# KangWelly/Assignment-for-AAE6102_GNSS-SDR

Hardware: NVIDIA B200
Metric: search cells/s (PRN x Doppler x code-phase), 32-PRN acquisition (higher is better)
Workload: dtype f32

## Files before the change

### assignment-for-aae6102_gnss-sdr_b200/csrc/gnss_kernels.cuh

```cuda
#pragma once
#include <cooperative_groups.h>
#include <climits>
#include "gnss_internal.h"

namespace gnss {
namespace cg = cooperative_groups;

struct NaturalLoader {
    static constexpr bool kStreams = false;
    const cf* __restrict__ in;
    template <int Q>
    __device__ __forceinline__ void load(int a, int b, cf (&z)[Q]) const {
        static_for<0, Q>([&](auto c_) {
            constexpr int C = decltype(c_)::value;
            z[C] = in[Geo<Q>::good(a, b, C)];
        });
    }
};
struct NaturalStorer {
    cf* __restrict__ out;
    template <int Q, int R>
    __device__ __forceinline__ void store2(int col, int, const cf (&w0)[16], const cf (&w1)[16]) {
        static_for<0, 16>([&](auto i_) {
            constexpr int I = decltype(i_)::value;
            constexpr int AP = (I / 4) + 4 * (I % 4);
            out[Geo<Q>::lag_of(AP, col)] = w0[I];
            if (col + 1 < Geo<Q>::ROW) out[Geo<Q>::lag_of(AP, col + 1)] = w1[I];
        });
    }
};

template <int R>
__device__ __forceinline__ void cl_arrive() {
    if constexpr (R > 1) asm volatile("barrier.cluster.arrive.release.aligned;" ::: "memory");
}
template <int R>
__device__ __forceinline__ void cl_wait() {
    if constexpr (R > 1) asm volatile("barrier.cluster.wait.acquire.aligned;" ::: "memory");
    else __syncthreads();
}
template <int R>
__device__ __forceinline__ void cl_sync() {
    cl_arrive<R>();
    cl_wait<R>();
}

template <int Q, int R, int T>
__device__ __forceinline__ void pass2_all(cf* D, const Tw4* tw, int tid) {
    pass2_cta<Q, R, T>(tid, D, tw);
}

template <int Q, int R, int T>
__device__ __forceinline__ void pass3_all(cf* D, const Tw4* tw, int tid) {
    using S = Split<Q, R>;
    (void)tw;
    for (int t = tid; t < S::P3_TASKS; t += T) pass3_task<Q, R>(t, D);
}

struct RedScratch {
    float wv[32];
    int wm[32];
    double ws[32];
    float peak; int lag; double sum_all; double sum_win;
    float g_peak; int g_lag;
};

template <int Q, int R>
struct Smem {
    using S = Split<Q, R>;
    static constexpr size_t d_bytes = (size_t)S::D_ELEMS * sizeof(cf);
    static constexpr size_t acc_floats = S::ACC_ELEMS > SplitX<Q, R>::ACC_ELEMS ? S::ACC_ELEMS : SplitX<Q, R>::ACC_ELEMS;
    static constexpr size_t acc_bytes = acc_floats * sizeof(float);
    static constexpr size_t tw_bytes = 100 * sizeof(Tw4);
    static constexpr size_t red_bytes = ((sizeof(RedScratch) + 15) / 16) * 16;
    static constexpr size_t transform = d_bytes + tw_bytes;
    static constexpr size_t search = d_bytes + acc_bytes + tw_bytes + red_bytes;
};

__device__ __forceinline__ void fill_tw125(Tw4* tw, int tid, int T) {
    for (int j = tid; j < 100; j += T) {
        double s, c;
        sincospi(-2.0 * (double)((j >> 2) * ((j & 3) + 1)) / 125.0, &s, &c);
        Tw4 w;
        w.c = (float)c; w.pad = 0.f; w.ns = -(float)s; w.s = (float)s;
        tw[j] = w;
    }
}

template <int T>
__device__ __forceinline__ void block_reduce(float& v, int& m, double& s, RedScratch* rs) {
    constexpr unsigned full = 0xffffffffu;
    constexpr int NW = T / 32;
#pragma unroll
    for (int off = 16; off; off >>= 1) {
        const float ov = __shfl_down_sync(full, v, off);
        const int om = __shfl_down_sync(full, m, off);
        const double os = __shfl_down_sync(full, s, off);
        if (peak_better(ov, om, v, m)) { v = ov; m = om; }
        s += os;
    }
    const int warp = threadIdx.x >> 5, lane = threadIdx.x & 31;
    if (lane == 0) { rs->wv[warp] = v; rs->wm[warp] = m; rs->ws[warp] = s; }
    __syncthreads();
    if (warp == 0) {
        v = lane < NW ? rs->wv[lane] : -1.f;
        m = lane < NW ? rs->wm[lane] : INT_MAX;
        s = lane < NW ? rs->ws[lane] : 0.0;
#pragma unroll
        for (int off = 16; off; off >>= 1) {
            const float ov = __shfl_down_sync(full, v, off);
            const int om = __shfl_down_sync(full, m, off);
            const double os = __shfl_down_sync(full, s, off);
            if (peak_better(ov, om, v, m)) { v = ov; m = om; }
            s += os;
        }
    }
    __syncthreads();
}

template <int Q, int R, int T, class Loader, class Storer>
__device__ __forceinline__ void unit_device(const Loader& ld, Storer& st, cf* D, cf* const* Dall,
                                            const Tw4* tw, int rank, int tid) {
    using S = Split<Q, R>;
    for (int t = tid; t < S::P1_TASKS; t += T) pass1_task<Q, R>(t, rank, ld, D);
    __syncthreads();
    pass2_all<Q, R, T>(D, tw, tid);
    __syncthreads();
    pass3_all<Q, R, T>(D, tw, tid);
    cl_sync<R>();
    for (int t = tid; t < S::P4_TASKS; t += T) pass4_task<Q, R>(t, rank, Dall, st);
    cl_sync<R>();
}

template <int Q, int R, int T, class Loader, class Storer>
__device__ __forceinline__ void unit_device_pipelined(const Loader& ld, Storer& st, cf* D, cf* const* Dall,
                                                      const Tw4* tw, int rank, int tid) {
    using S = Split<Q, R>;
    {
        cf z[Q];
        const bool has = tid < S::P1_TASKS;
        if (has) pass1_compute<Q, R>(tid, rank, ld, z);
        cl_wait<R>();
        if (has) pass1_store<Q, R>(tid, z, D);
    }
    for (int t = tid + T; t < S::P1_TASKS; t += T) pass1_task<Q, R>(t, rank, ld, D);
    __syncthreads();
    pass2_all<Q, R, T>(D, tw, tid);
    __syncthreads();
    pass3_all<Q, R, T>(D, tw, tid);
    cl_sync<R>();
    for (int t = tid; t < S::P4_TASKS; t += T) pass4_task<Q, R>(t, rank, Dall, st);
    cl_arrive<R>();
}

#define GNSS_KERNEL_PROLOGUE                                                     \
    using S = Split<Q, R>;                                                       \
    using G = Geo<Q>;                                                            \
    (void)sizeof(G);                                                             \
    cg::cluster_group cluster = cg::this_cluster();                              \
    const int tid = threadIdx.x;                                                 \
    const int rank = (R > 1) ? (int)cluster.block_rank() : 0;                    \
    const int unit = blockIdx.x / R;                                             \
    extern __shared__ __align__(16) unsigned char smem_raw[];                    \
    cf* D = reinterpret_cast<cf*>(smem_raw);                                     \
    cf* Dall[R];                                                                 \
    _Pragma("unroll") for (int r = 0; r < R; ++r)                                \
        Dall[r] = (R > 1) ? cluster.map_shared_rank(D, r) : D;

template <int Q, int R, int T, int MINB>
__global__ void __launch_bounds__(T, MINB) code_kernel(CodeArgs a) {
    GNSS_KERNEL_PROLOGUE
    Tw4* tw = reinterpret_cast<Tw4*>(D + S::D_ELEMS);
    fill_tw125(tw, tid, T);
    __syncthreads();
    CodeLoader ld{a.scode + (size_t)unit * G::N};
    SpectrumStorer st{a.cc + (size_t)unit * G::N, 1.0f / (float)G::N, 1, 0};
    unit_device<Q, R, T>(ld, st, D, Dall, tw, rank, tid);
}

template <int Q, int R, int T, int MINB>
__global__ void __launch_bounds__(T, MINB) wipe_kernel(WipeArgs a) {
    GNSS_KERNEL_PROLOGUE
    Tw4* tw = reinterpret_cast<Tw4*>(D + S::D_ELEMS);
    fill_tw125(tw, tid, T);
    __syncthreads();
    const int base = unit / a.K, k = unit - base * a.K;
    WipeoffLoader ld;
    ld.raw = (const unsigned char*)a.raw + (size_t)k * a.block_bytes;
    ld.data_type = a.data_type;
    ld.precision = a.precision;
    ld.coh_ms = a.coh_ms;
    ld.f_hz = a.base_freq_hz[base];
    ld.fs_hz = a.fs_hz;
    ld.mean_i = a.means ? (float)a.means[0] : 0.f;
    ld.mean_q = a.means ? (float)a.means[1] : 0.f;
    SpectrumStorer st{a.x + (size_t)unit * G::NX, 1.0f, 0, 1};
    unit_device<Q, R, T>(ld, st, D, Dall, tw, rank, tid);
}

__device__ __forceinline__ void cp_async16(void* smem_dst, const void* gmem_src) {
    const unsigned d = (unsigned)__cvta_generic_to_shared(smem_dst);
    asm volatile("cp.async.cg.shared.global [%0], [%1], 16;" ::"r"(d), "l"(gmem_src) : "memory");
}
__device__ __forceinline__ void cp_async_commit() { asm volatile("cp.async.commit_group;" ::: "memory"); }
template <int N_>
__device__ __forceinline__ void cp_async_wait() { asm volatile("cp.async.wait_group %0;" ::"n"(N_) : "memory"); }

template <int Q>
GNSS_HD int comb_row_of(int a) { return (a * (Geo<Q>::M1 % 16)) % 16; }

template <int Q, int R, int T, int MINB>
__global__ void __launch_bounds__(T, MINB) wipe2_kernel(Wipe2Args a) {
    GNSS_KERNEL_PROLOGUE
    Tw4* tw = reinterpret_cast<Tw4*>(D + S::D_ELEMS);
    unsigned char* stage = reinterpret_cast<unsigned char*>(tw + 100);
    fill_tw125(tw, tid, T);
    const int base = unit / a.K, k = unit - base * a.K;
    const double w = a.base_w[base];
    const float mean_i = a.means ? (float)a.means[0] : 0.f, mean_q = a.means ? (float)a.means[1] : 0.f;
    const int pitch = a.pitch, bps = a.bps, M = a.coh_ms;
    auto stage_ms = [&](int j, int buf) {
        const int chunks = pitch >> 4;
        for (int i = tid; i < S::A * chunks; i += T) {
            const int al = i / chunks, ch = i - al * chunks;
            const int rho = comb_row_of<Q>(rank * S::A + al);
            const unsigned char* src = a.comb + ((size_t)((size_t)k * M + j) * 16 + rho) * pitch + (size_t)ch * 16;
            cp_async16(stage + ((size_t)buf * S::A + al) * pitch + (size_t)ch * 16, src);
        }
        cp_async_commit();
    };
    constexpr int ROUNDS = (S::P1_TASKS + T - 1) / T;
    const int n_steps = (M > 1) ? ROUNDS * M : 1;
    stage_ms(0, 0);
    int step = 0;
    for (int t0 = 0; t0 < S::P1_TASKS; t0 += T) {
        const int task = t0 + tid;
        const bool has = task < S::P1_TASKS;
        const int al = has ? task / 125 : 0, b = has ? task - al * 125 : 0;
        const int arow = rank * S::A + al;
        cf z[Q];
        static_for<0, Q>([&](auto c_) { z[decltype(c_)::value] = mk(0.f, 0.f); });
        for (int j = 0; j < M; ++j) {
            const int buf = (M > 1) ? (step & 1) : 0;
            if (M > 1 || t0 == 0) {
                if (step + 1 < n_steps) { stage_ms((j + 1) % M, buf ^ 1); cp_async_wait<1>(); }
                else cp_async_wait<0>();
                __syncthreads();
            }
            if (has) {
                const unsigned char* row = stage + ((size_t)buf * S::A + al) * pitch;
                static_for<0, Q>([&](auto c_) {
                    constexpr int C = decltype(c_)::value;
                    const int n = Geo<Q>::good(arow, b, C);
                    const int m = n >> 4;
                    float xi, xq;
                    if (bps == 2) {
                        const unsigned short v = *reinterpret_cast<const unsigned short*>(row + 2 * m);
                        xi = (float)(signed char)(v & 0xff);
                        xq = (float)(signed char)(v >> 8);
                    } else if (bps == 4) {
                        const unsigned v = *reinterpret_cast<const unsigned*>(row + 4 * m);
                        xi = (float)(short)(v & 0xffff) - mean_i;
                        xq = (float)(short)(v >> 16) - mean_q;
                    } else {
                        xi = (float)(signed char)row[m];
                        xq = 0.f;
                    }
                    const double cyc = w * (double)((long long)j * Geo<Q>::N + n + 1);
                    const float fr = (float)(cyc - floor(cyc));
                    float si, co;
                    sincospif(2.0f * fr, &si, &co);
                    z[C].x += xi * co - xq * si;
                    z[C].y += xi * si + xq * co;
                });
            }
            if (M > 1) __syncthreads();
            ++step;
        }
        if (has) {
            dft_odd<Q>(z);
            pass1_store<Q, R>(task, z, D);
        }
    }
    cp_async_wait<0>();
    __syncthreads();
    pass2_all<Q, R, T>(D, tw, tid);
    __syncthreads();
    pass3_all<Q, R, T>(D, tw, tid);
    cl_sync<R>();
    SpectrumStorer st{a.x + (size_t)unit * G::NX, 1.0f, 0, 1};
    for (int t = tid; t < S::P4_TASKS; t += T) pass4_task<Q, R>(t, rank, Dall, st);
    cl_sync<R>();
}

template <int Q, int R, int T, int MINB>
__global__ void __launch_bounds__(T, MINB) natural_kernel(NaturalArgs a) {
    GNSS_KERNEL_PROLOGUE
    Tw4* tw = reinterpret_cast<Tw4*>(D + S::D_ELEMS);
    fill_tw125(tw, tid, T);
    __syncthreads();
    NaturalLoader ld{a.in + (size_t)unit * G::N};
    NaturalStorer st{a.out + (size_t)unit * G::N};
    unit_device<Q, R, T>(ld, st, D, Dall, tw, rank, tid);
}

template <int Q, int R, int T, int MINB>
__global__ void __launch_bounds__(T, MINB) fine_kernel(FineArgs a) {
    GNSS_KERNEL_PROLOGUE
    Tw4* tw = reinterpret_cast<Tw4*>(D + S::D_ELEMS);
    fill_tw125(tw, tid, T);
    __syncthreads();
    const int n2 = unit % a.L, r = (unit / a.L) % a.K, sv = unit / (a.L * a.K);
    FineLoader ld;
    ld.raw = a.raw;
    ld.chip = a.chip;
    ld.ca = a.ca + (size_t)sv * 1023;
    ld.data_type = a.data_type;
    ld.precision = a.precision;
    ld.mean_i = a.means ? (float)a.means[0] : 0.f;
    ld.mean_q = a.means ? (float)a.means[1] : 0.f;
    ld.start = a.start[sv];
    ld.L = a.L;
    ld.n2 = n2;
    ld.r = r;
    ld.F = a.F;
    NaturalStorerHD st{a.u + (size_t)unit * G::N};
    unit_device<Q, R, T>(ld, st, D, Dall, tw, rank, tid);
}

template <int Q, int R, int T, int MINB>
__global__ void __launch_bounds__(T, MINB) search_kernel(SearchArgs a) {
    GNSS_KERNEL_PROLOGUE
    float* acc = reinterpret_cast<float*>(D + S::D_ELEMS);
    Tw4* tw = reinterpret_cast<Tw4*>(acc + Smem<Q, R>::acc_floats);
    RedScratch* rs = reinterpret_cast<RedScratch*>(tw + 100);
    const int row = a.rows ? a.rows[unit] : a.row_first + unit;
    const int p = row % a.P, b = row / a.P;

    fill_tw125(tw, tid, T);
    for (int e = tid; e < S::ACC_ELEMS; e += T) acc[e] = 0.f;
    __syncthreads();

    int sa, sb, sc;
    G::shift_coords(a.bin_shift[b], sa, sb, sc);
    const cf* ccp = a.cc + (size_t)p * G::N;
    const cf* xb = a.x + (size_t)a.bin_base[b] * a.K * G::NX;
    PowerAccumStorer st{acc};
    cl_arrive<R>();
    for (int k = 0; k < a.K; ++k) {
        SearchLoader ld{ccp, xb + (size_t)k * G::NX, sa, sb, sc};
        unit_device_pipelined<Q, R, T>(ld, st, D, Dall, tw, rank, tid);
    }
    cl_wait<R>();

    float bv = -1.f;
    int bm = INT_MAX;
    double ss = 0.0;
    for (int e = tid; e < S::ACC_ELEMS; e += T) {
        const int ap = e / S::CH, t = e - ap * S::CH;
        const int col = rank * S::CH + t;
        if (col < S::ROW) {
            const float v = acc[e];
            const int m = G::lag_of(ap, col);
            if (peak_better(v, m, bv, bm)) { bv = v; bm = m; }
            ss += (double)v * (double)v;
            if (a.surface) a.surface[((size_t)p * a.B + b) * G::N + m] = v;
        }
    }
    block_reduce<T>(bv, bm, ss, rs);
    if (tid == 0) { rs->peak = bv; rs->lag = bm; rs->sum_all = ss; }
    if constexpr (R > 1) cluster.sync(); else __syncthreads();
    if (tid == 0) {
        float gv = -1.f;
        int gm = INT_MAX;
        for (int r = 0; r < R; ++r) {
            const RedScratch* o = (R > 1) ? cluster.map_shared_rank(rs, r) : rs;
            const float ov = o->peak;
            const int om = o->lag;
            if (peak_better(ov, om, gv, gm)) { gv = ov; gm = om; }
        }
        rs->g_peak = gv;
        rs->g_lag = gm;
    }
    __syncthreads();
    const int gm = rs->g_lag;
    double wsum = 0.0;
    for (int i = tid; i < 2 * a.w - 1; i += T) {
        const int m = gm - (a.w - 1) + i;
        if (m >= 0 && m < G::N) {
            int ap, col;
            G::cell_of_lag(m, ap, col);
            if (col / S::CH == rank) {
                const float v = acc[ap * S::CH + (col - rank * S::CH)];
                wsum += (double)v * (double)v;
            }
        }
    }
    float dv = -1.f;
    int dm = INT_MAX;
    block_reduce<T>(dv, dm, wsum, rs);
    if (tid == 0) rs->sum_win = wsum;
    if constexpr (R > 1) cluster.sync(); else __syncthreads();
    if (rank == 0 && tid == 0) {
        double s_all = 0.0, s_win = 0.0;
        for (int r = 0; r < R; ++r) {
            const RedScratch* o = (R > 1) ? cluster.map_shared_rank(rs, r) : rs;
            s_all += o->sum_all;
            s_win += o->sum_win;
        }
        Candidate c;
        c.peak = rs->g_peak;
        c.lag = rs->g_lag;
        c.sum_all = s_all;
        c.sum_win = s_win;
        a.cand[(size_t)p * a.cand_stride + b] = c;
    }
    if constexpr (R > 1) cluster.sync();
}

template <int Q, int R, int T, int MINB>
__global__ void __launch_bounds__(T, MINB) search_kernel_l2x(SearchArgs a) {
    GNSS_KERNEL_PROLOGUE
    (void)Dall;
    float* acc = reinterpret_cast<float*>(D + S::D_ELEMS);
    Tw4* tw = reinterpret_cast<Tw4*>(acc + Smem<Q, R>::acc_floats);
    RedScratch* rs = reinterpret_cast<RedScratch*>(tw + 100);
    const int ncl = gridDim.x / R, slot = unit;
    cf* xch = a.scratch + (size_t)slot * 2 * 16 * S::RS;
    fill_tw125(tw, tid, T);
    PowerAccumStorer st{acc};

    for (int lrow = slot; lrow < a.n_rows; lrow += ncl) {
        const int row = a.rows ? a.rows[lrow] : a.row_first + lrow;
        const int p = row % a.P, b = row / a.P;
        for (int e = tid; e < S::ACC_ELEMS; e += T) acc[e] = 0.f;
        int sa, sb, sc;
        G::shift_coords(a.bin_shift[b], sa, sb, sc);
        const cf* ccp = a.cc + (size_t)p * G::N;
        const cf* xb = a.x + (size_t)a.bin_base[b] * a.K * G::NX;
        {
            SearchLoader ld{ccp, xb, sa, sb, sc};
            for (int t = tid; t < S::P1_TASKS; t += T) pass1_task<Q, R>(t, rank, ld, D);
        }
        __syncthreads();
        pass2_all<Q, R, T>(D, tw, tid);
        __syncthreads();
        pass3_all<Q, R, T>(D, tw, tid);
        for (int k = 0; k < a.K; ++k) {
            const bool more = k + 1 < a.K;
            cf* buf = xch + (size_t)(k & 1) * 16 * S::RS;
            __syncthreads();
            {
                const float4* src = reinterpret_cast<const float4*>(D);
                float4* dst = reinterpret_cast<float4*>(buf + (size_t)rank * S::A * S::RS);
                for (int i = tid; i < S::D_ELEMS / 2; i += T) dst[i] = src[i];
            }
            if (more) {
                SearchLoader ld{ccp, xb + (size_t)(k + 1) * G::NX, sa, sb, sc};
                cf z[Q];
                const bool has = tid < S::P1_TASKS;
                if (has) pass1_compute<Q, R>(tid, rank, ld, z);
                __syncthreads();
                if (has) pass1_store<Q, R>(tid, z, D);
                for (int t = tid + T; t < S::P1_TASKS; t += T) pass1_task<Q, R>(t, rank, ld, D);
            }
            cl_arrive<R>();
            if (more) {
                __syncthreads();
                pass2_all<Q, R, T>(D, tw, tid);
            }
            cl_wait<R>();
            for (int t = tid; t < S::P4_TASKS; t += T) pass4_task_flat<Q, R>(t, rank, buf, st);
            if (more) {
                __syncthreads();
                pass3_all<Q, R, T>(D, tw, tid);
            }
        }
        __syncthreads();

        float bv = -1.f;
        int bm = INT_MAX;
        double ss = 0.0;
        for (int e = tid; e < S::ACC_ELEMS; e += T) {
            const int ap = e / S::CH, t = e - ap * S::CH;
            const int col = rank * S::CH + t;
            if (col < S::ROW) {
                const float v = acc[e];
                const int m = G::lag_of(ap, col);
                if (peak_better(v, m, bv, bm)) { bv = v; bm = m; }
                ss += (double)v * (double)v;
                if (a.surface) a.surface[((size_t)p * a.B + b) * G::N + m] = v;
            }
        }
        block_reduce<T>(bv, bm, ss, rs);
        if (tid == 0) { rs->peak = bv; rs->lag = bm; rs->sum_all = ss; }
        if constexpr (R > 1) cluster.sync(); else __syncthreads();
        if (tid == 0) {
            float gv = -1.f;
            int gm = INT_MAX;
            for (int r = 0; r < R; ++r) {
                const RedScratch* o = (R > 1) ? cluster.map_shared_rank(rs, r) : rs;
                const float ov = o->peak;
                const int om = o->lag;
                if (peak_better(ov, om, gv, gm)) { gv = ov; gm = om; }
            }
            rs->g_peak = gv;
            rs->g_lag = gm;
        }
        __syncthreads();
        const int gm = rs->g_lag;
        double wsum = 0.0;
        for (int i = tid; i < 2 * a.w - 1; i += T) {
            const int m = gm - (a.w - 1) + i;
            if (m >= 0 && m < G::N) {
                int ap, col;
                G::cell_of_lag(m, ap, col);
                if (col / S::CH == rank) {
                    const float v = acc[ap * S::CH + (col - rank * S::CH)];
                    wsum += (double)v * (double)v;
                }
            }
        }
        float dv = -1.f;
        int dm = INT_MAX;
        block_reduce<T>(dv, dm, wsum, rs);
        if (tid == 0) rs->sum_win = wsum;
        if constexpr (R > 1) cluster.sync(); else __syncthreads();
        if (rank == 0 && tid == 0) {
            double s_all = 0.0, s_win = 0.0;
            for (int r = 0; r < R; ++r) {
                const RedScratch* o = (R > 1) ? cluster.map_shared_rank(rs, r) : rs;
                s_all += o->sum_all;
                s_win += o->sum_win;
            }
            Candidate c;
            c.peak = rs->g_peak;
            c.lag = rs->g_lag;
            c.sum_all = s_all;
            c.sum_win = s_win;
            a.cand[(size_t)p * a.cand_stride + b] = c;
        }
        if constexpr (R > 1) cluster.sync(); else __syncthreads();
    }
}

__device__ __forceinline__ void group_arrive(unsigned* ctr) {
#ifdef GNSS_EXPERIMENT_NOFENCE
    asm volatile("red.relaxed.gpu.global.add.u32 [%0], 1;" ::"l"(ctr) : "memory");
#else
    asm volatile("red.release.gpu.global.add.u32 [%0], 1;" ::"l"(ctr) : "memory");
#endif
}
__device__ __forceinline__ void group_arrive_n(unsigned* ctr, unsigned n) {
    asm volatile("red.release.gpu.global.add.u32 [%0], %1;" ::"l"(ctr), "r"(n) : "memory");
}
__device__ __forceinline__ void group_spin(const unsigned* ctr, unsigned target) {
    unsigned v;
    do {
        asm volatile("ld.acquire.gpu.global.u32 %0, [%1];" : "=r"(v) : "l"(ctr) : "memory");
    } while ((int)(v - target) < 0);
}

template <int Q, int R, int T>
__device__ __noinline__ void publish_plane(float* acc, float* dst, int tid) {
    using SX = SplitX<Q, R>;
    for (int j = tid; j < SX::P4_TASKS; j += T) {
#pragma unroll
        for (int ap = 0; ap < 16; ++ap) {
            float2* p = reinterpret_cast<float2*>(acc + ap * SX::CHX + 2 * j);
            __stcg(reinterpret_cast<float2*>(dst + ap * SX::CHX + 2 * j), *p);
            *p = make_float2(0.f, 0.f);
        }
    }
}
template <int Q, int R, int T>
__device__ __noinline__ void merge_planes(float* acc, const float* planes, int n_planes, int tid) {
    constexpr int ACC4 = SplitX<Q, R>::ACC_ELEMS / 4;
    const float4* src = reinterpret_cast<const float4*>(planes);
    float4* a4 = reinterpret_cast<float4*>(acc);
    int q = tid;
    for (; q + T < ACC4; q += 2 * T) {
        float4 v = a4[q], w = a4[q + T];
#pragma unroll 4
        for (int k = 0; k < n_planes; ++k) {
            const float4 o = __ldcg(src + (size_t)k * (R * ACC4) + q);
            const float4 u = __ldcg(src + (size_t)k * (R * ACC4) + q + T);
            v.x += o.x; v.y += o.y; v.z += o.z; v.w += o.w;
            w.x += u.x; w.y += u.y; w.z += u.z; w.w += u.w;
        }
        a4[q] = v;
        a4[q + T] = w;
    }
    for (; q < ACC4; q += T) {
        float4 v = a4[q];
#pragma unroll 8
        for (int k = 0; k < n_planes; ++k) {
            const float4 o = __ldcg(src + (size_t)k * (R * ACC4) + q);
            v.x += o.x; v.y += o.y; v.z += o.z; v.w += o.w;
        }
        a4[q] = v;
    }
}

#ifdef GNSS_EXPERIMENT_NOBAR
#define GNSS_KSYNC() __syncwarp()
#else
#define GNSS_KSYNC() __syncthreads()
#endif
#ifdef GNSS_TIMELINE
#define GNSS_TL(i) do { if (tl_iter == 6 && group == 0 && (tid & 31) == 0) a.timeline[(rank * (T / 32) + (tid >> 5)) * 32 + (i)] = clock64(); } while (0)
#else
#define GNSS_TL(i) do { } while (0)
#endif
template <int Q, int R, int T, int MINB>
__global__ void __launch_bounds__(T, MINB) search_kernel_coop(SearchArgs a) {
    using S = Split<Q, R>;
    using G = Geo<Q>;
    using GX = GeoX<Q>;
    using SX = SplitX<Q, R>;
    const int tid = threadIdx.x;
    const int tid2 = (tid + T - 32) % T;
    const int tid3 = (tid + T - (64 % T)) % T;
    const int rank = blockIdx.x % R, group = blockIdx.x / R, ngroups = gridDim.x / R;
    extern __shared__ __align__(16) unsigned char smem_raw[];
    cf* D = reinterpret_cast<cf*>(smem_raw);
    float* acc = reinterpret_cast<float*>(D + S::D_ELEMS);
    Tw4* tw = reinterpret_cast<Tw4*>(acc + Smem<Q, R>::acc_floats);
    RedScratch* rs = reinterpret_cast<RedScratch*>(tw + 100);
    constexpr size_t XBUF = (size_t)16 * GX::RSX;
    cf* xch = a.scratch + (size_t)group * 2 * XBUF;
    unsigned* ctr = a.group_ctr + group;
    Candidate* slots = a.row_slots + (size_t)group * R;
    unsigned target = 0;
    fill_tw125(tw, tid, T);
    constexpr bool kRoomy = (T * MINB <= 512);
    constexpr bool kRegAcc = (Q <= 13) && kRoomy && (SX::P4_TASKS <= T);
    float racc0[16], racc1[16];
#pragma unroll
    for (int q = 0; q < 16; ++q) { racc0[q] = 0.f; racc1[q] = 0.f; }
    RegAccumStorer rst{racc0, racc1};
    PowerAccumStorer st{acc};
    auto dump_acc = [&]() {
        if constexpr (kRegAcc) {
            if (tid < SX::P4_TASKS) {
#pragma unroll
                for (int ap = 0; ap < 16; ++ap) {
                    *reinterpret_cast<float2*>(acc + ap * SX::CHX + 2 * tid) = make_float2(racc0[ap], racc1[ap]);
                    racc0[ap] = 0.f; racc1[ap] = 0.f;
                }
            }
        }
    };
    const int n_rows = a.n_rows;
    auto loader_of = [&](int lrow) {
        const int row = a.rows ? a.rows[lrow] : a.row_first + lrow;
        const int p = row % a.P, b = row / a.P;
        int sa, sb, sc;
        G::shift_coords(a.bin_shift[b], sa, sb, sc);
        return SearchLoader{a.cc + (size_t)p * G::N, a.x + (size_t)a.bin_base[b] * a.K * G::NX, sa, sb, sc};
    };
    const int full = n_rows / ngroups, tail_base = full * ngroups, n_tail = n_rows - tail_base;
    auto tb = [&](int g) -> int {
        return a.row_granular ? (g < n_tail ? g : n_tail) * a.K : (int)((unsigned)g * (unsigned)(n_tail * a.K) / (unsigned)ngroups);
    };
    struct Part { int row, kb, ke; };
    auto part = [&](int i) -> Part {
        if (i < full) return Part{i * ngroups + group, 0, a.K};
        const int t0 = tb(group), t1 = tb(group + 1), r0 = t0 / a.K, e0 = min(t1, (r0 + 1) * a.K);
        if (i == full) return Part{tail_base + r0, t0 - r0 * a.K, e0 - r0 * a.K};
        return Part{tail_base + r0 + 1, 0, t1 - e0};
    };
    auto count_parts = [&]() -> int {
        const int t0 = tb(group), t1 = tb(group + 1);
        return full + (t0 < t1 ? 1 + (min(t1, (t0 / a.K + 1) * a.K) < t1) : 0);
    };
    if (count_parts() == 0) return;
    int i = 0, par = 0;
    const Part first = part(0);
    int left = first.ke - first.kb;
    bool later = first.kb > 0;
    for (int e = tid; e < SX::ACC_ELEMS; e += T) acc[e] = 0.f;
    SearchLoader ld = loader_of(first.row);
    ld.x += (size_t)first.kb * G::NX;
    for (int t = tid; t < S::P1_TASKS; t += T) pass1_task<Q, R>(t, rank, ld, D);
    __syncthreads();
    pass2_all<Q, R, T>(D, tw, tid2);
    __syncthreads();
    for (int t = tid3; t < S::P3_TASKS; t += T) pass3_task_xt<Q, R>(t, D, xch + (size_t)rank * S::A * GX::RSX);
#ifdef GNSS_TIMELINE
    int tl_iter = 0;
#endif
    for (;;) {
#ifdef GNSS_TIMELINE
        ++tl_iter;
#endif
        GNSS_TL(0);
        const bool last_of_part = (left == 1);
        const bool more = !last_of_part || i + 1 < count_parts();
        const cf* buf = xch + (size_t)par * XBUF;
        cf* nbuf = xch + (size_t)(par ^ 1) * XBUF;
        par ^= 1;
        target += R;
        if (more) {
            if (last_of_part) {
                const Part np = part(i + 1);
                ld = loader_of(np.row);
                ld.x += (size_t)np.kb * G::NX;
            } else {
                ld.x += G::NX;
            }
            cf z[Q];
            const bool has = tid < S::P1_TASKS;
            if (has) pass1_compute<Q, R>(tid, rank, ld, z);
            constexpr bool kTwo = (Q <= 13) && kRoomy && (S::P1_TASKS > T) && (S::P1_TASKS <= 2 * T);
            cf z2[kTwo ? Q : 1];
            const bool has2 = kTwo && tid + T < S::P1_TASKS;
            if constexpr (kTwo) { if (has2) pass1_compute<Q, R>(tid + T, rank, ld, z2); }
            GNSS_TL(1);
            GNSS_KSYNC();
            GNSS_TL(2);
            if (tid == 0) group_arrive(ctr);
            GNSS_TL(3);
            if (has) pass1_store<Q, R>(tid, z, D);
            if constexpr (kTwo) {
                if (has2) pass1_store<Q, R>(tid + T, z2, D);
            } else if constexpr (S::P1_TASKS > T) {
                for (int t = tid + T; t < S::P1_TASKS; t += T) pass1_task<Q, R>(t, rank, ld, D);
            }
            GNSS_TL(4);
            GNSS_KSYNC();
            GNSS_TL(5);
            pass2_all<Q, R, T>(D, tw, tid2);
            GNSS_TL(6);
        } else {
            GNSS_KSYNC();
            if (tid == 0) group_arrive(ctr);
        }
#ifndef GNSS_EXPERIMENT_NOSPIN
        if (tid == 0) group_spin(ctr, target);
#endif
        GNSS_TL(7);
        GNSS_KSYNC();
        GNSS_TL(8);
#pragma unroll 1
        for (int half = 0; half < 2; ++half) {
            const int flip = (((tid >> 5) + 1) >> 1) & 1;
            if ((half ^ flip) == 0) {
                if constexpr (kRegAcc) {
                    if (tid < SX::P4_TASKS) pass4_task_xt<Q, R>(tid, rank, buf, rst);
                } else {
                    for (int t = tid; t < SX::P4_TASKS; t += T) pass4_task_xt<Q, R>(t, rank, buf, st);
                }
            } else if (more) {
                for (int t = tid3; t < S::P3_TASKS; t += T) pass3_task_xt<Q, R>(t, D, nbuf + (size_t)rank * S::A * GX::RSX);
            }
        }
        GNSS_TL(10);
        if (later) {
            const Part cp = part(i);
            const int kk = cp.ke - left;
            int gf = group - 1;
            while (tb(gf) > (cp.row - tail_base) * a.K) --gf;
            float* dst = a.partial + (((size_t)gf * (a.K - 1) + (kk - 1)) * R + rank) * SX::ACC_ELEMS;
            dump_acc();
            publish_plane<Q, R, T>(acc, dst, tid);
            if (last_of_part) {
                __syncthreads();
                if (tid == 0) group_arrive_n(a.part_ctr + (size_t)gf * R + rank, (unsigned)(cp.ke - cp.kb));
            }
        } else if (last_of_part) {
            dump_acc();
            __syncthreads();
            const Part cp = part(i);
            const int row = cp.row;
            if (cp.ke < a.K) {
                if (tid == 0) group_spin(a.part_ctr + (size_t)group * R + rank, (unsigned)(a.K - cp.ke));
                __syncthreads();
                merge_planes<Q, R, T>(acc, a.partial + (((size_t)group * (a.K - 1) + (cp.ke - 1)) * R + rank) * SX::ACC_ELEMS,
                                      a.K - cp.ke, tid);
                __syncthreads();
            }
            const int grow = a.rows ? a.rows[row] : a.row_first + row, p = grow % a.P, b = grow / a.P;
            float bv = -1.f;
            int bm = INT_MAX;
            double ss = 0.0;
            if (a.surface) {
                for (int e = tid; e < SX::ACC_ELEMS; e += T) {
                    const int ap = e / SX::CHX, t = e - ap * SX::CHX;
                    const int ex = rank * SX::CHX + t;
                    if (GX::valid(ex)) {
                        const float v = acc[e];
                        const int m = GX::lag_of(ap, ex);
                        if (peak_better(v, m, bv, bm)) { bv = v; bm = m; }
                        ss += (double)v * (double)v;
                        a.surface[((size_t)p * a.B + b) * G::N + m] = v;
                    }
                }
            } else {
                const float4* a4 = reinterpret_cast<const float4*>(acc);
                for (int q = tid; q < SX::ACC_ELEMS / 4; q += T) {
                    const float4 v = a4[q];
                    ss += (double)v.x * v.x + (double)v.y * v.y + (double)v.z * v.z + (double)v.w * v.w;
                    const float vm = fmaxf(fmaxf(v.x, v.y), fmaxf(v.z, v.w));
                    if (vm >= bv) {
                        const float vv[4] = {v.x, v.y, v.z, v.w};
#pragma unroll
                        for (int u = 0; u < 4; ++u) {
                            const int e = 4 * q + u;
                            const int ap = e / SX::CHX, t = e - ap * SX::CHX;
                            const int ex = rank * SX::CHX + t;
                            if (vv[u] >= bv && GX::valid(ex)) {
                                const int m = GX::lag_of(ap, ex);
                                if (peak_better(vv[u], m, bv, bm)) { bv = vv[u]; bm = m; }
                            }
                        }
                    }
                }
            }
            block_reduce<T>(bv, bm, ss, rs);
            target += R;
            if (tid == 0) {
                Candidate c; c.peak = bv; c.lag = bm; c.sum_all = ss; c.sum_win = 0.0;
                slots[rank] = c;
                group_arrive(ctr);
                group_spin(ctr, target);
                float gv = -1.f;
                int gm = INT_MAX;
                for (int r = 0; r < R; ++r) {
                    const float ov = __ldcg(&slots[r].peak);
                    const int om = __ldcg(&slots[r].lag);
                    if (peak_better(ov, om, gv, gm)) { gv = ov; gm = om; }
                }
                rs->g_peak = gv;
                rs->g_lag = gm;
            }
            __syncthreads();
            const int gm = rs->g_lag;
            double wsum = 0.0;
            for (int i = tid; i < 2 * a.w - 1; i += T) {
                const int m = gm - (a.w - 1) + i;
                if (m >= 0 && m < G::N) {
                    int ap, ex;
                    GX::cell_of_lag(m, ap, ex);
                    if (ex / SX::CHX == rank) {
                        const float v = acc[ap * SX::CHX + (ex - rank * SX::CHX)];
                        wsum += (double)v * (double)v;
                    }
                }
            }
            float dv = -1.f;
            int dm = INT_MAX;
            block_reduce<T>(dv, dm, wsum, rs);
            if constexpr (!kRegAcc)
                for (int e = tid; e < SX::ACC_ELEMS; e += T) acc[e] = 0.f;
            if (tid == 0) {
                slots[rank].sum_win = wsum;
                unsigned old;
                asm volatile("atom.acq_rel.gpu.global.add.u32 %0, [%1], 1;" : "=r"(old) : "l"(a.row_ticket + group) : "memory");
                if ((old + 1) % R == 0) {
                    double s_all = 0.0, s_win = 0.0;
                    for (int r = 0; r < R; ++r) {
                        s_all += __ldcg(&slots[r].sum_all);
                        s_win += __ldcg(&slots[r].sum_win);
                    }
                    Candidate c;
                    c.peak = rs->g_peak;
                    c.lag = rs->g_lag;
                    c.sum_all = s_all;
                    c.sum_win = s_win;
                    a.cand[(size_t)p * a.cand_stride + b] = c;
                }
            }
        }
        if (!more) break;
        if (last_of_part) {
            const Part np = part(++i);
            left = np.ke - np.kb;
            later = np.kb > 0;
        } else {
            --left;
        }
    }
}

template <class K, class A>
static cudaError_t launch_clustered(K kern, const A& args, int units, int R, int T, size_t smem, cudaStream_t s) {
    cudaLaunchConfig_t cfg = {};
    cfg.gridDim = dim3((unsigned)(units * R), 1, 1);
    cfg.blockDim = dim3((unsigned)T, 1, 1);
    cfg.dynamicSmemBytes = smem;
    cfg.stream = s;
    cudaLaunchAttribute attr[1];
    attr[0].id = cudaLaunchAttributeClusterDimension;
    attr[0].val.clusterDim.x = (unsigned)R;
    attr[0].val.clusterDim.y = 1;
    attr[0].val.clusterDim.z = 1;
    cfg.attrs = attr;
    cfg.numAttrs = 1;
    A copy = args;
    return cudaLaunchKernelEx(&cfg, kern, copy);
}

template <int Q, int R, int T, int MINB>
struct Variant {
    static constexpr int RT = R > 8 ? 8 : R;
    static constexpr int TT = R > 8 ? 256 : T;
    static constexpr int MT = R > 8 ? 2 : MINB;
    static cudaError_t prepare() {
        cudaError_t e;
        e = cudaFuncSetAttribute(code_kernel<Q, RT, TT, MT>, cudaFuncAttributeMaxDynamicSharedMemorySize, (int)Smem<Q, RT>::transform);
        if (e != cudaSuccess) return e;
        e = cudaFuncSetAttribute(wipe_kernel<Q, RT, TT, MT>, cudaFuncAttributeMaxDynamicSharedMemorySize, (int)Smem<Q, RT>::transform);
        if (e != cudaSuccess) return e;
        e = cudaFuncSetAttribute(wipe2_kernel<Q, RT, TT, MT>, cudaFuncAttributeMaxDynamicSharedMemorySize, 227 * 1024);
        if (e != cudaSuccess) return e;
        e = cudaFuncSetAttribute(natural_kernel<Q, RT, TT, MT>, cudaFuncAttributeMaxDynamicSharedMemorySize, (int)Smem<Q, RT>::transform);
        if (e != cudaSuccess) return e;
        e = cudaFuncSetAttribute(fine_kernel<Q, RT, TT, MT>, cudaFuncAttributeMaxDynamicSharedMemorySize, (int)Smem<Q, RT>::transform);
        if (e != cudaSuccess) return e;
        e = cudaFuncSetAttribute(search_kernel_coop<Q, R, T, MINB>, cudaFuncAttributeMaxDynamicSharedMemorySize, (int)Smem<Q, R>::search);
        if (e != cudaSuccess) return e;

        e = cudaFuncSetAttribute(search_kernel_l2x<Q, R, T, MINB>, cudaFuncAttributeMaxDynamicSharedMemorySize, (int)Smem<Q, R>::search);
        if (e != cudaSuccess) return e;
        return cudaFuncSetAttribute(search_kernel<Q, R, T, MINB>, cudaFuncAttributeMaxDynamicSharedMemorySize, (int)Smem<Q, R>::search);
    }
    static cudaError_t launch_search_l2x(const SearchArgs& a, int clusters, cudaStream_t s) {
        if (R > 8) return cudaErrorInvalidConfiguration;
        return launch_clustered(search_kernel_l2x<Q, R, T, MINB>, a, clusters, R, T, Smem<Q, R>::search, s);
    }
    static cudaError_t launch_search_coop(const SearchArgs& a, int groups, cudaStream_t s) {
        SearchArgs copy = a;
        void* args[] = {&copy};
        return cudaLaunchCooperativeKernel((const void*)search_kernel_coop<Q, R, T, MINB>, dim3((unsigned)(groups * R)),
                                           dim3((unsigned)T), args, Smem<Q, R>::search, s);
    }
    static int max_groups_coop() {
        int per_sm = 0, dev = 0, sms = 0;
        if (cudaOccupancyMaxActiveBlocksPerMultiprocessor(&per_sm, search_kernel_coop<Q, R, T, MINB>, T, Smem<Q, R>::search) != cudaSuccess) { cudaGetLastError(); return 0; }
        cudaGetDevice(&dev);
        cudaDeviceGetAttribute(&sms, cudaDevAttrMultiProcessorCount, dev);
        return per_sm * sms / R;
    }
    static int max_clusters_l2x() {
        cudaLaunchConfig_t cfg = {};
        cfg.gridDim = dim3((unsigned)(R * 1024), 1, 1);
        cfg.blockDim = dim3((unsigned)T, 1, 1);
        cfg.dynamicSmemBytes = Smem<Q, R>::search;
        cudaLaunchAttribute attr[1];
        attr[0].id = cudaLaunchAttributeClusterDimension;
        attr[0].val.clusterDim.x = (unsigned)R;
        attr[0].val.clusterDim.y = 1;
        attr[0].val.clusterDim.z = 1;
        cfg.attrs = attr;
        cfg.numAttrs = 1;
        int n = 0;
        if (cudaOccupancyMaxActiveClusters(&n, search_kernel_l2x<Q, R, T, MINB>, &cfg) != cudaSuccess) { cudaGetLastError(); return 0; }
        return n;
    }
    static cudaError_t launch_code(const CodeArgs& a, int units, cudaStream_t s) {
        return launch_clustered(code_kernel<Q, RT, TT, MT>, a, units, RT, TT, Smem<Q, RT>::transform, s);
    }
    static cudaError_t launch_wipe(const WipeArgs& a, int units, cudaStream_t s) {
        return launch_clustered(wipe_kernel<Q, RT, TT, MT>, a, units, RT, TT, Smem<Q, RT>::transform, s);
    }
    static size_t smem_wipe2(int pitch, int coh_ms) {
        return Smem<Q, RT>::transform + (size_t)(coh_ms > 1 ? 2 : 1) * Split<Q, RT>::A * (size_t)pitch;
    }
    static cudaError_t launch_wipe2(const Wipe2Args& a, int units, cudaStream_t s) {
        return launch_clustered(wipe2_kernel<Q, RT, TT, MT>, a, units, RT, TT, smem_wipe2(a.pitch, a.coh_ms), s);
    }
    static cudaError_t launch_natural(const NaturalArgs& a, int units, cudaStream_t s) {
        return launch_clustered(natural_kernel<Q, RT, TT, MT>, a, units, RT, TT, Smem<Q, RT>::transform, s);
    }
    static cudaError_t launch_fine(const FineArgs& a, int units, cudaStream_t s) {
        return launch_clustered(fine_kernel<Q, RT, TT, MT>, a, units, RT, TT, Smem<Q, RT>::transform, s);
    }
    static cudaError_t launch_search(const SearchArgs& a, int rows, cudaStream_t s) {
        if (R > 8) return cudaErrorInvalidConfiguration;
        return launch_clustered(search_kernel<Q, R, T, MINB>, a, rows, R, T, Smem<Q, R>::search, s);
    }
    static constexpr VariantOps ops() {
        return VariantOps{Q, R, T, Smem<Q, R>::search, Smem<Q, RT>::transform,
                          &prepare, &launch_code, &launch_wipe, &launch_wipe2, &smem_wipe2, &launch_natural, &launch_fine, &launch_search,
                          &launch_search_l2x, &max_clusters_l2x,
                          (size_t)2 * 16 * (Split<Q, R>::RS > GeoX<Q>::RSX ? Split<Q, R>::RS : GeoX<Q>::RSX) * sizeof(cf),
                          &launch_search_coop, &max_groups_coop,
                          (size_t)R * SplitX<Q, R>::ACC_ELEMS * sizeof(float)};
    }
};

}
```

Measured before the change: 10.76 billion.

## Pack four warpgroups per CTA and cache pass-1 code samples in TMEM

The cooperative search kernel can now run W=4 independent 128-thread warpgroups per CTA, each with its own shared-memory slice and named barriers in place of __syncthreads. Each warpgroup also gets 128 TMEM columns. During pass 1 it writes the code replica samples to tensor memory on the first block of a partition and reads them back from TMEM on later blocks, so they are not reloaded from global memory each time. This mode is used only when K is at least 4 and the launch config is T=128, MINB=4. It adds tcgen05 allocation and fence overhead, and occupancy is limited to the minimum of the W=1 and W=4 variants.

```diff
diff --git a/assignment-for-aae6102_gnss-sdr_b200/csrc/gnss_kernels.cuh b/assignment-for-aae6102_gnss-sdr_b200/csrc/gnss_kernels.cuh
--- a/assignment-for-aae6102_gnss-sdr_b200/csrc/gnss_kernels.cuh
+++ b/assignment-for-aae6102_gnss-sdr_b200/csrc/gnss_kernels.cuh
@@ -87,8 +87,14 @@
     }
 }
 
-template <int T>
-__device__ __forceinline__ void block_reduce(float& v, int& m, double& s, RedScratch* rs) {
+template <int T, int W>
+__device__ __forceinline__ void wg_sync(int wg) {
+    if constexpr (W == 1) __syncthreads();
+    else asm volatile("bar.sync %0, %1;" ::"r"(1 + wg), "n"(T) : "memory");
+}
+
+template <int T, int W = 1>
+__device__ __forceinline__ void block_reduce(float& v, int& m, double& s, RedScratch* rs, int wg = 0) {
     constexpr unsigned full = 0xffffffffu;
     constexpr int NW = T / 32;
 #pragma unroll
@@ -99,9 +105,9 @@
         if (peak_better(ov, om, v, m)) { v = ov; m = om; }
         s += os;
     }
-    const int warp = threadIdx.x >> 5, lane = threadIdx.x & 31;
+    const int warp = (threadIdx.x % T) >> 5, lane = threadIdx.x & 31;
     if (lane == 0) { rs->wv[warp] = v; rs->wm[warp] = m; rs->ws[warp] = s; }
-    __syncthreads();
+    wg_sync<T, W>(wg);
     if (warp == 0) {
         v = lane < NW ? rs->wv[lane] : -1.f;
         m = lane < NW ? rs->wm[lane] : INT_MAX;
@@ -115,7 +121,7 @@
             s += os;
         }
     }
-    __syncthreads();
+    wg_sync<T, W>(wg);
 }
 
 template <int Q, int R, int T, class Loader, class Storer>
@@ -544,6 +550,70 @@
     }
 }
 
+__device__ __forceinline__ void tmem_st2(uint32_t t, cf u) {
+    asm volatile("tcgen05.st.sync.aligned.32x32b.x2.b32 [%0], {%1, %2};" ::"r"(t), "f"(u.x), "f"(u.y));
+}
+__device__ __forceinline__ void tmem_st4(uint32_t t, cf u, cf v) {
+    asm volatile("tcgen05.st.sync.aligned.32x32b.x4.b32 [%0], {%1, %2, %3, %4};" ::"r"(t), "f"(u.x), "f"(u.y), "f"(v.x), "f"(v.y));
+}
+__device__ __forceinline__ void tmem_ld2(uint32_t t, float (&r)[2]) {
+    asm volatile("tcgen05.ld.sync.aligned.32x32b.x2.b32 {%0, %1}, [%2];" : "=f"(r[0]), "=f"(r[1]) : "r"(t));
+}
+__device__ __forceinline__ void tmem_ld4(uint32_t t, float (&r)[4]) {
+    asm volatile("tcgen05.ld.sync.aligned.32x32b.x4.b32 {%0, %1, %2, %3}, [%4];" : "=f"(r[0]), "=f"(r[1]), "=f"(r[2]), "=f"(r[3]) : "r"(t));
+}
+__device__ __forceinline__ void tmem_wait_ld(float (&r)[4]) {
+    asm volatile("tcgen05.wait::ld.sync.aligned;" : "+f"(r[0]), "+f"(r[1]), "+f"(r[2]), "+f"(r[3]));
+}
+__device__ __forceinline__ void tmem_wait_ld(float (&r)[2], float (&u)[4]) {
+    asm volatile("tcgen05.wait::ld.sync.aligned;" : "+f"(r[0]), "+f"(r[1]), "+f"(u[0]), "+f"(u[1]), "+f"(u[2]), "+f"(u[3]));
+}
+__device__ __forceinline__ void tmem_wait_st() { asm volatile("tcgen05.wait::st.sync.aligned;" ::: "memory"); }
+
+template <int Q>
+constexpr int kTmemStripCols = 4 + 4 * ((Q - 1) / 2);
+
+template <int Q, int R, bool kFill>
+__device__ __forceinline__ void pass1_compute_tmem(int task, int rank, const SearchLoader& ld, uint32_t t, cf (&z)[Q]) {
+    using S = Split<Q, R>;
+    constexpr int H = (Q - 1) / 2;
+    const int al = task / 125, b = task - al * 125;
+    const auto ctx = ld.template begin<Q>(rank * S::A + al, b);
+    if constexpr (kFill) {
+        cf held = mk(0.f, 0.f);
+        dft_odd_stream<Q>([&](auto cc) {
+            constexpr int C = decltype(cc)::value;
+            const cf c = ld_ro(ctx.pc + C * 125);
+            if constexpr (C == 0) tmem_st2(t, c);
+            else if constexpr (C <= H) held = c;
+            else tmem_st4(t + 4 * (Q - C), held, c);
+            return cmul_scalar(c, ld_ro(ctx.px + C * 125));
+        }, z);
+    } else {
+        float c0[2], cur[4], nxt[4];
+        tmem_wait_st();
+        tmem_ld2(t, c0);
+        tmem_ld4(t + 4, cur);
+        tmem_wait_ld(c0, cur);
+        dft_odd_stream<Q>([&](auto cc) {
+            constexpr int C = decltype(cc)::value;
+            if constexpr (C == 0) {
+                return cmul_scalar(mk(c0[0], c0[1]), ld_ro(ctx.px));
+            } else if constexpr (C <= H) {
+                if constexpr (C > 1) {
+                    tmem_wait_ld(nxt);
+#pragma unroll
+                    for (int i = 0; i < 4; ++i) cur[i] = nxt[i];
+                }
+                if constexpr (C < H) tmem_ld4(t + 4 * (C + 1), nxt);
+                return cmul_scalar(mk(cur[0], cur[1]), ld_ro(ctx.px + C * 125));
+            } else {
+                return cmul_scalar(mk(cur[2], cur[3]), ld_ro(ctx.px + C * 125));
+            }
+        }, z);
+    }
+}
+
 __device__ __forceinline__ void group_arrive(unsigned* ctr) {
 #ifdef GNSS_EXPERIMENT_NOFENCE
     asm volatile("red.relaxed.gpu.global.add.u32 [%0], 1;" ::"l"(ctr) : "memory");
@@ -605,25 +675,28 @@
 #ifdef GNSS_EXPERIMENT_NOBAR
 #define GNSS_KSYNC() __syncwarp()
 #else
-#define GNSS_KSYNC() __syncthreads()
+#define GNSS_KSYNC() wg_sync<T, W>(wg)
 #endif
 #ifdef GNSS_TIMELINE
 #define GNSS_TL(i) do { if (tl_iter == 6 && group == 0 && (tid & 31) == 0) a.timeline[(rank * (T / 32) + (tid >> 5)) * 32 + (i)] = clock64(); } while (0)
 #else
 #define GNSS_TL(i) do { } while (0)
 #endif
-template <int Q, int R, int T, int MINB>
-__global__ void __launch_bounds__(T, MINB) search_kernel_coop(SearchArgs a) {
+template <int Q, int R, int T, int MINB, int W>
+__device__ __forceinline__ void search_coop_wg(const SearchArgs& a, int tid, int wg, unsigned char* smem, uint32_t tmem) {
     using S = Split<Q, R>;
     using G = Geo<Q>;
     using GX = GeoX<Q>;
     using SX = SplitX<Q, R>;
-    const int tid = threadIdx.x;
     const int tid2 = (tid + T - 32) % T;
     const int tid3 = (tid + T - (64 % T)) % T;
-    const int rank = blockIdx.x % R, group = blockIdx.x / R, ngroups = gridDim.x / R;
-    extern __shared__ __align__(16) unsigned char smem_raw[];
-    cf* D = reinterpret_cast<cf*>(smem_raw);
+#ifdef GNSS_EXPERIMENT_GROUP_PER_CTA
+    const int v = (int)blockIdx.x * W + wg;
+#else
+    const int v = wg * (int)gridDim.x + (int)blockIdx.x;
+#endif
+    const int rank = v % R, group = v / R, ngroups = (int)gridDim.x * W / R;
+    cf* D = reinterpret_cast<cf*>(smem);
     float* acc = reinterpret_cast<float*>(D + S::D_ELEMS);
     Tw4* tw = reinterpret_cast<Tw4*>(acc + Smem<Q, R>::acc_floats);
     RedScratch* rs = reinterpret_cast<RedScratch*>(tw + 100);
@@ -635,6 +708,10 @@
     fill_tw125(tw, tid, T);
     constexpr bool kRoomy = (T * MINB <= 512);
     constexpr bool kRegAcc = (Q <= 13) && kRoomy && (SX::P4_TASKS <= T);
+    constexpr bool kTwo = (Q <= 13) && kRoomy && (S::P1_TASKS > T) && (S::P1_TASKS <= 2 * T);
+    constexpr bool kTmem = (W > 1) && (S::P1_TASKS <= T || kTwo);
+    constexpr int kSlots = (S::P1_TASKS + T - 1) / T;
+    static_assert(!kTmem || kSlots * kTmemStripCols<Q> <= 128, "a warpgroup owns 128 TMEM columns");
     float racc0[16], racc1[16];
 #pragma unroll
     for (int q = 0; q < 16; ++q) { racc0[q] = 0.f; racc1[q] = 0.f; }
@@ -650,6 +727,11 @@
                 }
             }
         }
+    };
+    auto pass1_tmem = [&](bool fill, const SearchLoader& l, int slot, cf (&zz)[Q]) {
+        const int t = min(tid + slot * T, S::P1_TASKS - 1);
+        if (fill) pass1_compute_tmem<Q, R, true>(t, rank, l, tmem + slot * kTmemStripCols<Q>, zz);
+        else pass1_compute_tmem<Q, R, false>(t, rank, l, tmem + slot * kTmemStripCols<Q>, zz);
     };
     const int n_rows = a.n_rows;
     auto loader_of = [&](int lrow) {
@@ -682,10 +764,19 @@
     for (int e = tid; e < SX::ACC_ELEMS; e += T) acc[e] = 0.f;
     SearchLoader ld = loader_of(first.row);
     ld.x += (size_t)first.kb * G::NX;
-    for (int t = tid; t < S::P1_TASKS; t += T) pass1_task<Q, R>(t, rank, ld, D);
-    __syncthreads();
+    if constexpr (kTmem) {
+#pragma unroll 1
+        for (int slot = 0; slot < kSlots; ++slot) {
+            cf z[Q];
+            pass1_tmem(true, ld, slot, z);
+            if (tid + slot * T < S::P1_TASKS) pass1_store<Q, R>(tid + slot * T, z, D);
+        }
+    } else {
+        for (int t = tid; t < S::P1_TASKS; t += T) pass1_task<Q, R>(t, rank, ld, D);
+    }
+    wg_sync<T, W>(wg);
     pass2_all<Q, R, T>(D, tw, tid2);
-    __syncthreads();
+    wg_sync<T, W>(wg);
     for (int t = tid3; t < S::P3_TASKS; t += T) pass3_task_xt<Q, R>(t, D, xch + (size_t)rank * S::A * GX::RSX);
 #ifdef GNSS_TIMELINE
     int tl_iter = 0;
@@ -711,11 +802,15 @@
             }
             cf z[Q];
             const bool has = tid < S::P1_TASKS;
-            if (has) pass1_compute<Q, R>(tid, rank, ld, z);
-            constexpr bool kTwo = (Q <= 13) && kRoomy && (S::P1_TASKS > T) && (S::P1_TASKS <= 2 * T);
             cf z2[kTwo ? Q : 1];
             const bool has2 = kTwo && tid + T < S::P1_TASKS;
-            if constexpr (kTwo) { if (has2) pass1_compute<Q, R>(tid + T, rank, ld, z2); }
+            if constexpr (kTmem) {
+                pass1_tmem(last_of_part, ld, 0, z);
+                if constexpr (kTwo) pass1_tmem(last_of_part, ld, 1, z2);
+            } else {
+                if (has) pass1_compute<Q, R>(tid, rank, ld, z);
+                if constexpr (kTwo) { if (has2) pass1_compute<Q, R>(tid + T, rank, ld, z2); }
+            }
             GNSS_TL(1);
             GNSS_KSYNC();
             GNSS_TL(2);
@@ -765,20 +860,20 @@
             dump_acc();
             publish_plane<Q, R, T>(acc, dst, tid);
             if (last_of_part) {
-                __syncthreads();
+                wg_sync<T, W>(wg);
                 if (tid == 0) group_arrive_n(a.part_ctr + (size_t)gf * R + rank, (unsigned)(cp.ke - cp.kb));
             }
         } else if (last_of_part) {
             dump_acc();
-            __syncthreads();
+            wg_sync<T, W>(wg);
             const Part cp = part(i);
             const int row = cp.row;
             if (cp.ke < a.K) {
                 if (tid == 0) group_spin(a.part_ctr + (size_t)group * R + rank, (unsigned)(a.K - cp.ke));
-                __syncthreads();
+                wg_sync<T, W>(wg);
                 merge_planes<Q, R, T>(acc, a.partial + (((size_t)group * (a.K - 1) + (cp.ke - 1)) * R + rank) * SX::ACC_ELEMS,
                                       a.K - cp.ke, tid);
-                __syncthreads();
+                wg_sync<T, W>(wg);
             }
             const int grow = a.rows ? a.rows[row] : a.row_first + row, p = grow % a.P, b = grow / a.P;
             float bv = -1.f;
@@ -817,7 +912,7 @@
                     }
                 }
             }
-            block_reduce<T>(bv, bm, ss, rs);
+            block_reduce<T, W>(bv, bm, ss, rs, wg);
             target += R;
             if (tid == 0) {
                 Candidate c; c.peak = bv; c.lag = bm; c.sum_all = ss; c.sum_win = 0.0;
@@ -834,7 +929,7 @@
                 rs->g_peak = gv;
                 rs->g_lag = gm;
             }
-            __syncthreads();
+            wg_sync<T, W>(wg);
             const int gm = rs->g_lag;
             double wsum = 0.0;
             for (int i = tid; i < 2 * a.w - 1; i += T) {
@@ -850,7 +945,7 @@
             }
             float dv = -1.f;
             int dm = INT_MAX;
-            block_reduce<T>(dv, dm, wsum, rs);
+            block_reduce<T, W>(dv, dm, wsum, rs, wg);
             if constexpr (!kRegAcc)
                 for (int e = tid; e < SX::ACC_ELEMS; e += T) acc[e] = 0.f;
             if (tid == 0) {
@@ -883,6 +978,37 @@
     }
 }
 
+template <int Q, int R, int T, int MINB, int W>
+__global__ void __launch_bounds__(T * W, MINB / W) search_kernel_coop(SearchArgs a) {
+    static_assert(R % W == 0 && MINB % W == 0, "a CTA holds whole groups' worth of warpgroups");
+    static_assert(Smem<Q, R>::search % 16 == 0, "warpgroup slices stay 16-byte aligned");
+    extern __shared__ __align__(16) unsigned char smem_raw[];
+    const int wg = (int)threadIdx.x / T;
+    unsigned char* smem = smem_raw + (size_t)wg * Smem<Q, R>::search;
+    if constexpr (W == 1) {
+        search_coop_wg<Q, R, T, MINB, W>(a, (int)threadIdx.x, 0, smem, 0u);
+    } else {
+        static_assert(W * 128 <= 512, "TMEM columns");
+        __shared__ uint32_t tmem_base;
+        const bool warp0 = threadIdx.x < 32;
+        if (warp0) {
+            asm volatile("tcgen05.alloc.cta_group::1.sync.aligned.shared::cta.b32 [%0], 512;"
+                         ::"r"((uint32_t)__cvta_generic_to_shared(&tmem_base)) : "memory");
+            asm volatile("tcgen05.relinquish_alloc_permit.cta_group::1.sync.aligned;" ::: "memory");
+        }
+        asm volatile("tcgen05.fence::before_thread_sync;" ::: "memory");
+        __syncthreads();
+        asm volatile("tcgen05.fence::after_thread_sync;" ::: "memory");
+        const uint32_t tmem = tmem_base + ((threadIdx.x & 96u) << 16) + (uint32_t)(128 * wg);
+        search_coop_wg<Q, R, T, MINB, W>(a, (int)threadIdx.x % T, wg, smem, tmem);
+        tmem_wait_st();
+        asm volatile("tcgen05.fence::before_thread_sync;" ::: "memory");
+        __syncthreads();
+        asm volatile("tcgen05.fence::after_thread_sync;" ::: "memory");
+        if (warp0) asm volatile("tcgen05.dealloc.cta_group::1.sync.aligned.b32 %0, 512;" ::"r"(tmem_base) : "memory");
+    }
+}
+
 template <class K, class A>
 static cudaError_t launch_clustered(K kern, const A& args, int units, int R, int T, size_t smem, cudaStream_t s) {
     cudaLaunchConfig_t cfg = {};
@@ -903,6 +1029,23 @@
 
 template <int Q, int R, int T, int MINB>
 struct Variant {
+    static constexpr int W = (T == 128 && MINB == 4 && R % 4 == 0) ? 4 : 1;
+    static constexpr int kFusedMinK = 4;
+    template <int Wk>
+    static cudaError_t launch_coop(const SearchArgs& a, int groups, cudaStream_t s) {
+        SearchArgs copy = a;
+        void* args[] = {&copy};
+        return cudaLaunchCooperativeKernel((const void*)search_kernel_coop<Q, R, T, MINB, Wk>, dim3((unsigned)(groups * R / Wk)),
+                                           dim3((unsigned)(T * Wk)), args, Wk * Smem<Q, R>::search, s);
+    }
+    template <int Wk>
+    static int groups_coop() {
+        int per_sm = 0, dev = 0, sms = 0;
+        if (cudaOccupancyMaxActiveBlocksPerMultiprocessor(&per_sm, search_kernel_coop<Q, R, T, MINB, Wk>, T * Wk, Wk * Smem<Q, R>::search) != cudaSuccess) { cudaGetLastError(); return 0; }
+        cudaGetDevice(&dev);
+        cudaDeviceGetAttribute(&sms, cudaDevAttrMultiProcessorCount, dev);
+        return per_sm * sms * Wk / R;
+    }
     static constexpr int RT = R > 8 ? 8 : R;
     static constexpr int TT = R > 8 ? 256 : T;
     static constexpr int MT = R > 8 ? 2 : MINB;
@@ -918,8 +1061,12 @@
         if (e != cudaSuccess) return e;
         e = cudaFuncSetAttribute(fine_kernel<Q, RT, TT, MT>, cudaFuncAttributeMaxDynamicSharedMemorySize, (int)Smem<Q, RT>::transform);
         if (e != cudaSuccess) return e;
-        e = cudaFuncSetAttribute(search_kernel_coop<Q, R, T, MINB>, cudaFuncAttributeMaxDynamicSharedMemorySize, (int)Smem<Q, R>::search);
+        e = cudaFuncSetAttribute(search_kernel_coop<Q, R, T, MINB, 1>, cudaFuncAttributeMaxDynamicSharedMemorySize, (int)Smem<Q, R>::search);
         if (e != cudaSuccess) return e;
+        if constexpr (W > 1) {
+            e = cudaFuncSetAttribute(search_kernel_coop<Q, R, T, MINB, W>, cudaFuncAttributeMaxDynamicSharedMemorySize, (int)(W * Smem<Q, R>::search));
+            if (e != cudaSuccess) return e;
+        }
 
         e = cudaFuncSetAttribute(search_kernel_l2x<Q, R, T, MINB>, cudaFuncAttributeMaxDynamicSharedMemorySize, (int)Smem<Q, R>::search);
         if (e != cudaSuccess) return e;
@@ -930,17 +1077,15 @@
         return launch_clustered(search_kernel_l2x<Q, R, T, MINB>, a, clusters, R, T, Smem<Q, R>::search, s);
     }
     static cudaError_t launch_search_coop(const SearchArgs& a, int groups, cudaStream_t s) {
-        SearchArgs copy = a;
-        void* args[] = {&copy};
-        return cudaLaunchCooperativeKernel((const void*)search_kernel_coop<Q, R, T, MINB>, dim3((unsigned)(groups * R)),
-                                           dim3((unsigned)T), args, Smem<Q, R>::search, s);
+        if constexpr (W > 1) {
+            if (a.K >= kFusedMinK) return launch_coop<W>(a, groups, s);
+        }
+        return launch_coop<1>(a, groups, s);
     }
     static int max_groups_coop() {
-        int per_sm = 0, dev = 0, sms = 0;
-        if (cudaOccupancyMaxActiveBlocksPerMultiprocessor(&per_sm, search_kernel_coop<Q, R, T, MINB>, T, Smem<Q, R>::search) != cudaSuccess) { cudaGetLastError(); return 0; }
-        cudaGetDevice(&dev);
-        cudaDeviceGetAttribute(&sms, cudaDevAttrMultiProcessorCount, dev);
-        return per_sm * sms / R;
+        const int n = groups_coop<1>();
+        if constexpr (W > 1) return min(n, groups_coop<W>());
+        return n;
     }
     static int max_clusters_l2x() {
         cudaLaunchConfig_t cfg = {};
diff --git a/profiles/ab_tmem.py b/profiles/ab_tmem.py
--- /dev/null
+++ b/profiles/ab_tmem.py
@@ -0,0 +1,74 @@
+import os
+import subprocess
+import sys
+
+HERE = os.path.dirname(os.path.abspath(__file__))
+CHILD = r'''
+import ctypes, hashlib, os, sys
+sys.path.insert(0, os.environ["AB_PROFILES"])
+import explib
+explib.use_lib(os.environ["AB_LIB"])
+import gnssacq
+from gnssacq import api
+from gnssacq.synth import urban_recording, opensky_recording
+for which, rec, fs, if_hz in (("q29", opensky_recording, 58e6, 4.58e6), ("q13", urban_recording, 26e6, 0.0)):
+    for k in [int(x) for x in sys.argv[2].split(",")]:
+        raw = rec().read(0, k)
+        for n in [int(x) for x in sys.argv[1].split(",")]:
+            cfg = gnssacq.make_config(fs_hz=fs, if_hz=if_hz, prns=range(1, n + 1), noncoh_blocks=k)
+            with api.Searcher(cfg) as s:
+                best = 1e9
+                for _ in range(8):
+                    rows = s.search(raw)
+                    best = min(best, s.last_stats.search_ms)
+                st = s.last_stats
+                digest = hashlib.sha1(b"".join(ctypes.string_at(ctypes.addressof(r), ctypes.sizeof(r)) for r in rows)).hexdigest()[:10]
+            print(which + "k" + str(k), n, round(best, 4), digest, st.resident_clusters, flush=True)
+'''
+
+
+def main():
+    libs = [a.split("=", 1) for a in sys.argv[1:] if "=" in a and not a.startswith("--")]
+    prns, ks, rounds = "32", "20", 3
+    for i, a in enumerate(sys.argv):
+        if a == "--prns":
+            prns = sys.argv[i + 1]
+        if a == "--k":
+            ks = sys.argv[i + 1]
+        if a == "--rounds":
+            rounds = int(sys.argv[i + 1])
+    times, digests, groups = {}, {}, {}
+    for r in range(rounds):
+        for name, path in libs:
+            env = dict(os.environ, AB_LIB=os.path.abspath(path), AB_PROFILES=HERE)
+            out = subprocess.run([sys.executable, "-c", CHILD, prns, ks], env=env, capture_output=True, text=True)
+            if out.returncode:
+                print(name, "FAILED", out.stderr[-800:], flush=True)
+                continue
+            for line in out.stdout.split("\n"):
+                if line.strip():
+                    which, n, ms, digest, res = line.split()
+                    key = (which, int(n), name)
+                    times.setdefault(key, []).append(float(ms))
+                    digests.setdefault(key, set()).add(digest)
+                    groups[key] = int(res)
+                    print("round", r, name, which, n, ms, digest, "groups", res, flush=True)
+    base = libs[0][0]
+    for which in [q + "k" + k for q in ("q29", "q13") for k in ks.split(",")]:
+        for n in [int(x) for x in prns.split(",")]:
+            b = times.get((which, n, base))
+            for name, _ in libs:
+                t = times.get((which, n, name))
+                if not t:
+                    continue
+                line = f"{which} prns {n} {name:>10}: " + " ".join(f"{x:.4f}" for x in t)
+                line += f"  mean {sum(t) / len(t):.4f}  spread {max(t) - min(t):.4f}  groups {groups[(which, n, name)]}"
+                line += f"  rows {','.join(sorted(digests[(which, n, name)]))}"
+                if b and len(b) == len(t):
+                    d = [100.0 * (y / x - 1.0) for x, y in zip(b, t)]
+                    line += "  vs " + base + " per round " + " ".join(f"{x:+.2f}%" for x in d)
+                print(line, flush=True)
+
+
+if __name__ == "__main__":
+    main()
```

Measured after the change: 11.11 billion (median of 6 runs). 1.03x the previous value.
